# mic-rud/Learned-Compression-of-Point-Cloud-Geometry-and-Attributes

Hardware: AMD Instinct MI355X
Metric: encode+decode Mpoints/sec (higher is better)
Workload: dtype f32

## Files before the change

### include/pcc_hip.h

```cpp
#ifndef PCC_HIP_H
#define PCC_HIP_H

#include <stdint.h>

#ifdef __cplusplus
extern "C" {
#endif

#define PCC_OK 0
#define PCC_ERR_ARG (-1)
#define PCC_ERR_HIP (-2)
#define PCC_ERR_UNSUPPORTED (-3)
#define PCC_ERR_DATA (-4)

#define PCC_ACT_NONE 0
#define PCC_ACT_RELU 1
#define PCC_ACT_LEAKY_RELU 2

int pcc_version(void);
const char* pcc_last_error(void);
int pcc_device_count(void);
int pcc_device_name(int dev, char* out, int out_len);

int64_t pcc_hash_capacity(int64_t n);
// ... 43 lines not shown
int pcc_order_rows_by_mask(const uint32_t* row_mask, const int32_t* coords, int64_t n,
                           int32_t block_log2, int32_t tensor_stride, int32_t* order, uint32_t* group_mask32,
                           void* scratch, int64_t scratch_bytes, void* stream);
int pcc_permute_map_rows(const int32_t* nbr, const int32_t* order, int64_t n, int32_t K, int32_t* nbr_sorted, void* stream);

int64_t pcc_small_map_max(void);
int32_t pcc_small_paths(int32_t mask);
int pcc_small_kernel_map(const int32_t* out_coords, int64_t n_out, const uint64_t* in_keys, const int32_t* in_vals, int64_t in_cap,
                         int32_t ksize, int32_t step, int32_t sign, int32_t* nbr, uint32_t* row_mask, int32_t* order,
                         uint32_t* group_mask32, void* scratch, int64_t scratch_bytes, void* stream);

int64_t pcc_conv_packed_elems(int32_t K, int32_t cin, int32_t cout);
int pcc_conv_pack_weights(const float* w, int32_t K, int32_t cin, int32_t cout, float* w_packed,
                          void* stream);
int pcc_conv_fwd(const float* fin, int64_t n_in, int32_t cin, const float* w, const float* w_packed,
                 const float* bias, const int32_t* nbr, const int32_t* order,
                 const uint32_t* group_mask32, int32_t K, float* fout, int64_t n_out, int32_t cout,
                 int32_t act, const float* film, const float* residual, void* stream);

int64_t pcc_conv_small_max(int64_t workgroups);

int pcc_conv_kernel_name(int32_t mode, int64_t n_in, int32_t cin, int32_t cout, int64_t n_out, int32_t K, int32_t has_nbr,
                         char* buf, int32_t len);

int64_t pcc_conv_packed_elems_bf16(int32_t K, int32_t cin, int32_t cout);
int pcc_conv_pack_weights_bf16(const float* w, int32_t K, int32_t cin, int32_t cout, uint16_t* w_packed, void* stream);
int pcc_conv_fwd_bf16(const uint16_t* fin, int64_t n_in, int32_t cin, const uint16_t* w_packed, const float* bias,
                      const int32_t* nbr, const int32_t* order, const uint32_t* group_mask32, int32_t K, float* fout,
                      int64_t n_out, int32_t cout, int32_t act, const float* film, const float* residual, void* stream);

int pcc_epilogue_fwd(const float* c, const float* film, const float* residual, int64_t n, int32_t channels, int32_t act,
                     float* out, void* stream);
int pcc_epilogue_bwd(const float* dout, const float* c, const float* film, int64_t n, int32_t channels, int32_t act,
                     float* dc, float* dfilm, void* stream);

int64_t pcc_cast_colsum_scratch_elems(int32_t channels);
int pcc_cast_colsum(const float* x, int64_t n, int32_t channels, uint16_t* out_bf16, float* colsum, float* scratch,
                    int64_t scratch_elems, void* stream);

int64_t pcc_conv_packed_elems_x3(int32_t K, int32_t cin, int32_t cout);
int pcc_conv_pack_weights_x3(const float* w, int32_t K, int32_t cin, int32_t cout, uint16_t* w_packed, void* stream);
int pcc_conv_fwd_x3(const float* fin, int64_t n_in, int32_t cin, const uint16_t* w_packed, const float* bias,
                    const int32_t* nbr, const int32_t* order, const uint32_t* group_mask32, int32_t K, float* fout,
                    int64_t n_out, int32_t cout, int32_t act, const float* film, const float* residual, void* stream);

int pcc_im2col_thin(const float* fin, int32_t cin, const int32_t* nbr, int64_t n_out, int32_t K, float* out, int32_t k2,
// ... 146 lines not shown
```

### learned-compression-of-point-cloud-geometry-and-attributes_amd/_build.py

```python
import os
import subprocess

_HERE = os.path.dirname(os.path.abspath(__file__))
SO_PATH = os.path.join(_HERE, "libpcc_hip.so")

NO_SCRATCH = {
    "conv": ("conv_small_kernel", "conv_mfma_buf_kernel", "conv_mfma_kernel"),
    "rans_lanes": ("rans_lanes_encode_kernel", "rans_lanes_pack_kernel", "rans_lanes_decode_kernel"),
    "chconv": ("chconv_kernel",),
    "augment": ("jitter_partial_kernel", "jitter_mean_kernel", "jitter_apply_kernel", "first_rows_clear_kernel",
                "first_rows_insert_kernel", "first_rows_flag_kernel", "first_rows_finalize_kernel"),
    "normals": ("estimate_normals_kernel",),
    "voxelize": ("first_rows_clear_kernel", "first_rows_insert_kernel", "first_rows_flag_kernel", "first_rows_finalize_kernel",
                 "voxelize_accumulate_kernel"),
    "raht": ("raht_plan_kernel", "raht_step_kernel", "raht_fold_kernel"),
}


def build(force=False):
    args = ["make", "-s", "-C", os.path.join(_HERE, "csrc"), "-j4"]
    if force:
        subprocess.check_call(args + ["clean"])
    subprocess.check_call(args)
    for stem, kernels in NO_SCRATCH.items():
        check_kernel_resources(os.path.join(_HERE, "build", stem + ".resources.txt"), kernels)
    check_small_kernel_lds_reads()
    return SO_PATH


def check_small_kernel_lds_reads(obj=None):
# ... 94 lines not shown
```

### learned-compression-of-point-cloud-geometry-and-attributes_amd/csrc/conv.hip

```cpp
#include <stdlib.h>

#include <type_traits>

#include "common.h"

namespace pcc {

typedef float f32x2 __attribute__((ext_vector_type(2)));
typedef float f32x4 __attribute__((ext_vector_type(4)));
typedef __bf16 bf16x8 __attribute__((ext_vector_type(8)));

struct ConvArgs {
    const float* fin;
    const float* w;
    const float* wp;
    const float* bias;
    const int32_t* nbr;
    const int32_t* order;
    const uint32_t* gmask;
    float* fout;
    const float* film;
    const float* residual;
    int64_t n_in, n_out;
    int cin, cout, coutp, K, act;
};

__device__ __forceinline__ float apply_act(float v, int act) {
    if (act == PCC_ACT_RELU) return v > 0.0f ? v : 0.0f;
    if (act == PCC_ACT_LEAKY_RELU) return v > 0.0f ? v : 0.01f * v;
    return v;
}

__device__ __forceinline__ float conv_bias(const ConvArgs& a, int col) { return a.bias ? a.bias[col] : 0.0f; }

__device__ __forceinline__ void conv_store(const ConvArgs& a, int64_t row, int col, float acc, float bcol) {
    float v = acc + bcol;
    if (a.film) {
        const float* fr = a.film + row * (2 * (int64_t)a.cout);
        v = v * fr[col] + fr[a.cout + col];
    }
    v = apply_act(v, a.act);
    if (a.residual) v += a.residual[row * a.cout + col];
    a.fout[row * a.cout + col] = v;
}

__global__ __launch_bounds__(256) void pack_weights_kernel(const float* __restrict__ w, int K, int cin, int cout,
                                                           int cinp, int coutp, float* __restrict__ wp) {
// ... 164 lines not shown
        else if (live == 2u) block(std::integral_constant<unsigned, 2u>{});
    }
}

template <int MT, int NT>
__device__ __forceinline__ void conv_store_tiles(const ConvArgs& a, const f32x16 (&acc)[MT][NT], int64_t pos0, int col0, int h) {
#pragma unroll
    for (int m = 0; m < MT; ++m) {
#pragma unroll
        for (int n = 0; n < NT; ++n) {
            const int col = col0 + 32 * n;
            if (col >= a.cout) continue;
            const float bcol = conv_bias(a, col);
#pragma unroll
            for (int reg = 0; reg < 16; ++reg) {
                const int64_t pos = pos0 + 32 * m + 4 * h + mfma32_row(reg);
                if (pos >= a.n_out) continue;
                conv_store(a, a.order ? a.order[pos] : pos, col, acc[m][n][reg], bcol);
            }
        }
    }
}

template <int BM, int BN, int WAVES_M, int WAVES_N, bool HAS_NBR>
__global__ __launch_bounds__(256) void conv_mfma_kernel(const ConvArgs a) {
    constexpr int RPT = BM / 32;
    constexpr int WM = BM / WAVES_M, WN = BN / WAVES_N;
    constexpr int MT = WM / 32, NT = WN / 32;
    constexpr int A_LD = A_LD_DMA;
    constexpr int A_ELEMS = BM * A_LD;
    constexpr int W_ELEMS = 8 * BN * 4;
    constexpr int W_LOADS = (8 * BN) / 256;
    static_assert(WAVES_M * WAVES_N == 4 && MT >= 1 && NT >= 1 && W_LOADS >= 1, "bad tiling");

    extern __shared__ __attribute__((aligned(16))) float smem[];
    float* As = smem;
    float* Ws = smem + 2 * A_ELEMS;

    const int t = threadIdx.x;
    const int lane = t & 63, wid = t >> 6;
    const int r = lane & 31, h = lane >> 5;
    const int wrow = (wid / WAVES_N) * WM, wcol = (wid % WAVES_N) * WN;

    const int ntiles_n = a.coutp / BN;
    const int64_t tile = blockIdx.x / ntiles_n;
    const int nt = blockIdx.x - (int)(tile * ntiles_n);
// ... 106 lines not shown
            compute(cur, k);
            __syncthreads();
            if (!has_next) break;
            if (advance) { k = nk; rem = rem2; knext = kn2; }
            c = nc;
            cur ^= 1;
        }
    }

    conv_store_tiles(a, acc, row0 + wrow, nt * BN + wcol + r, h);
}

constexpr uint32_t BUF_OOB = 0xFFFFF000u;
[[maybe_unused]] constexpr uint32_t BUF_FLAGS = 0x00020000u;

template <int I, int N, class F>
__device__ __forceinline__ void static_for(F&& f) {
    if constexpr (I < N) {
        f(std::integral_constant<int, I>{});
        static_for<I + 1, N>(f);
    }
}

template <int BM, int BN, int WAVES_M, int WAVES_N, int CCH, bool HAS_NBR, bool BF16 = false, bool X3 = false>
__global__ __launch_bounds__(256) void conv_mfma_buf_kernel(const ConvArgs a) {
#if defined(__HIP_DEVICE_COMPILE__)
    constexpr int RPT = BM / 32;
    constexpr int WM = BM / WAVES_M, WN = BN / WAVES_N;
    constexpr int MT = WM / 32, NT = WN / 32;
    constexpr int A_ELEMS = BM * 32;
    constexpr int W_ELEMS = (X3 ? 12 : 8) * BN * 4;
    constexpr int W_LOADS = ((X3 ? 12 : 8) * BN) / 256;
    static_assert(WAVES_M * WAVES_N == 4 && MT >= 1 && MT <= 2 && NT >= 1 && W_LOADS >= 1, "bad tiling");
    static_assert(!(BF16 && X3), "one operand mode at a time");
    constexpr int ESZ = BF16 ? 2 : 4;

    extern __shared__ __attribute__((aligned(16))) float smem[];
    float* As = smem;
    float* Ws = smem + 2 * A_ELEMS;

    const int t = threadIdx.x;
    const int lane = t & 63, wid = t >> 6;
    const int r = lane & 31, h = lane >> 5;
    const int wrow = (wid / WAVES_N) * WM, wcol = (wid % WAVES_N) * WN;

    const int ntiles_n = a.coutp / BN;
    const int64_t tile = blockIdx.x / ntiles_n;
    const int nt = blockIdx.x - (int)(tile * ntiles_n);
// ... 167 lines not shown
                }
                compute(std::integral_constant<int, buf>{}, live);
                __syncthreads();
            });
            const bool more = knext >= 0;
            k = more ? knext : k;
            rem = rem2;
            return more;
        };

        load_idx(k);
        set_src(true);
        dma(k, std::integral_constant<int, 0>{}, std::integral_constant<int, 0>{});
        load_idx(rem ? __builtin_ctz(rem) : k);
        __syncthreads();
        while (true) {
            if (!offset_body(std::integral_constant<int, 0>{})) break;
            if constexpr (CCH & 1) {
                if (!offset_body(std::integral_constant<int, 1>{})) break;
            }
        }
    }

    conv_store_tiles(a, acc, row0 + wrow, nt * BN + wcol + r, h);
#endif
}

template <int SC, int NS>
constexpr int conv_small_lds_bytes() { return (NS * SC * (32 * 32 + 8 * 32 * 4) + 32 * 32) * (int)sizeof(float); }

template <int SC, int NS>
__global__ __launch_bounds__(512) void conv_small_kernel(const ConvArgs a) {
#if defined(__HIP_DEVICE_COMPILE__)
    constexpr int A_STAGE = SC * 32 * 32;
    constexpr int W_STAGE = SC * 8 * 32 * 4;
    constexpr int STAGE = A_STAGE + W_STAGE;
    constexpr int DMAS = 2 * SC;
    static_assert(NS >= 2 && (NS - 1) * DMAS <= 63, "vmcnt is a 6-bit counter");
    extern __shared__ __attribute__((aligned(16))) float smem[];
    int* idx_s = reinterpret_cast<int*>(smem + NS * STAGE);

    const int t = threadIdx.x;
    const int lane = t & 63;
    const int wave_u = __builtin_amdgcn_readfirstlane(t >> 6);
    const int K = a.K;
    const int ntiles_n = a.coutp / 32;
    const int64_t tile = blockIdx.x / ntiles_n;
// ... 272 lines not shown
        for (int u = 0; u < 9; ++u)
            if (idx[u] >= 0) {
#pragma unroll
                for (int c = 0; c < COUT; ++c) acc[c] += v[u][c];
            }
    }
    float* o = out + (row0 + threadIdx.x) * COUT;
#pragma unroll
    for (int c = 0; c < COUT; ++c) o[c] = apply_act(acc[c] + (bias ? bias[c] : 0.0f), act);
}

enum ConvMode { CONV_F32 = 0, CONV_BF16 = 1, CONV_X3 = 2 };
static const char* const CONV_ENTRY[] = {"pcc_conv_fwd", "pcc_conv_fwd_bf16", "pcc_conv_fwd_x3"};
static const char* const CONV_TAG[] = {"", "[bf16]", "[x3]"};

enum ConvFamily { FAM_THIN, FAM_SMALL, FAM_BUF, FAM_GLOBAL };

struct ConvPlan {
    ConvFamily family;
    int bm, bn, wm, wn;
    int cch;
    int sc, ns;
    int cpt;
};

constexpr int64_t FILL_WGS = 768;
constexpr int64_t ROW32_MAX_WGS = 3000;

static inline int round_up32(int v) { return (v + 31) / 32 * 32; }

static bool fits_buffer_path(const ConvArgs& a) {
    const uint64_t lim = BUF_OOB;
    return (uint64_t)a.n_in * a.cin * 4 <= lim && (uint64_t)a.n_out * a.K * 4 <= lim && (uint64_t)a.K * a.cin * a.coutp * 4 <= lim;
}

static int conv_path() {
    static int path = -1;
    if (path < 0) { const char* e = getenv("PCC_CONV_PATH"); path = (e && e[0] == 'g') ? 1 : 0; }
    return path;
}

static int64_t g_small_max = -1;
static int64_t small_max_value() {
    if (g_small_max < 0) { const char* e = getenv("PCC_CONV_SMALL_MAX"); g_small_max = e ? atoll(e) : 640; }
    return g_small_max;
}

static bool thin_cin(int cin) {
    for (int c : {1, 2, 3, 4, 6, 8, 12, 16, 24})
        if (cin == c) return true;
    return false;
}

static int check_shape(const ConvArgs& a, ConvMode mode, const char* who) {
    PCC_REQUIRE(a.K >= 1 && a.K <= 27, "%s: K=%d out of range", who, a.K);
    if (mode == CONV_F32) PCC_REQUIRE(a.cin % 32 != 0 || a.cin <= 256, "%s: MFMA path supports cin <= 256 (got %d)", who, a.cin);
    if (mode == CONV_BF16) PCC_REQUIRE(a.cin % 64 == 0 && a.cin <= 256, "%s: cin must be a multiple of 64 up to 256 (got %d)", who, a.cin);
    if (mode == CONV_X3) PCC_REQUIRE(a.cin % 32 == 0 && a.cin <= 256, "%s: cin must be a multiple of 32 up to 256 (got %d)", who, a.cin);
    PCC_REQUIRE(a.nbr != nullptr || (a.K == 1 && a.n_in == a.n_out), "%s: nbr == NULL needs K == 1 and n_in == n_out", who);
    return PCC_OK;
}

static int plan_conv(const ConvArgs& a, ConvMode mode, ConvPlan& p, const char* who) {
    p = ConvPlan{};
    if (mode == CONV_F32 && a.cin % 32 != 0) {
        if (!thin_cin(a.cin)) {
            pcc::set_error("%s: unsupported cin=%d (need a multiple of 32 or one of 1,2,3,4,6,8,12,16,24)", who, a.cin);
            return PCC_ERR_UNSUPPORTED;
        }
        const size_t lds = (size_t)a.K * a.cin * a.cout * sizeof(float);
        PCC_REQUIRE(lds <= 160 * 1024, "conv(thin): weights %zu B exceed the 160 KB of LDS (cin=%d cout=%d K=%d)", lds, a.cin, a.cout, a.K);
        p.family = FAM_THIN;
        p.cpt = (a.cout % 8 == 0) ? 8 : (a.cout % 4 == 0) ? 4 : (a.cout % 2 == 0) ? 2 : 1;
        return PCC_OK;
    }
    const bool wide = a.coutp % 128 == 0;
    p.family = FAM_BUF;
    p.cch = a.cin / (mode == CONV_BF16 ? 64 : 32);
    if (mode == CONV_F32) {
        const bool buffer = conv_path() == 0 && fits_buffer_path(a);
        const int64_t wgs32 = ((a.n_out + 31) / 32) * (a.coutp / 32);
        if (a.nbr && buffer && wgs32 <= small_max_value() * (wide ? 1 : 2)) {
            p.family = FAM_SMALL;
            p.sc = (p.cch % 4 == 0 && wgs32 <= 256) ? 4 : p.cch % 2 == 0 ? 2 : 1;
            p.ns = p.sc == 1 ? 8 : 3;
            return PCC_OK;
        }
        if (!buffer) p.family = FAM_GLOBAL;
    } else if (mode == CONV_BF16) {
        PCC_REQUIRE((uint64_t)a.n_in * a.cin * 2 <= BUF_OOB && (uint64_t)a.n_out * a.K * 4 <= BUF_OOB,
                    "%s: operands of 4 GiB and more are not supported", who);
    } else {
        PCC_REQUIRE((uint64_t)a.n_in * a.cin * 4 <= BUF_OOB && (uint64_t)a.n_out * a.K * 4 <= BUF_OOB &&
                    (uint64_t)a.K * a.cin * a.coutp * 6 <= BUF_OOB, "%s: operands of 4 GiB and more are not supported", who);
    }
    const int64_t wgs128 = ((a.n_out + 63) / 64) * (a.coutp / 128);
    auto tile = [&](int bm, int bn, int wm, int wn) { p.bm = bm; p.bn = bn; p.wm = wm; p.wn = wn; return PCC_OK; };
    if (wide && wgs128 < FILL_WGS) return tile(64, 64, 2, 2);
    if (wide && mode == CONV_F32 && wgs128 < ROW32_MAX_WGS) return tile(32, 128, 1, 4);
    if (wide) return tile(64, 128, 2, 2);
    if (a.coutp % 64 == 0) return mode == CONV_X3 ? tile(64, 64, 2, 2) : tile(128, 64, 2, 2);
    if (mode != CONV_X3) return tile(128, 32, 4, 1);
    pcc::set_error("%s: cout=%d not supported (output width rounded up to 32 must be a multiple of 64)", who, a.cout);
    return PCC_ERR_UNSUPPORTED;
}

template <auto KERN>
static int launch(int64_t blocks, int threads, size_t lds, size_t lds_limit, const ConvArgs& a, hipStream_t st) {
    static bool limit_set = false;
    if (lds_limit && !limit_set) {
        PCC_CHECK_HIP(hipFuncSetAttribute(reinterpret_cast<const void*>(KERN), hipFuncAttributeMaxDynamicSharedMemorySize, (int)lds_limit));
        limit_set = true;
    }
    PCC_REQUIRE(blocks < (1ll << 31), "conv: grid too large");
    hipLaunchKernelGGL(KERN, dim3((unsigned)blocks), dim3(threads), lds, st, a);
    PCC_LAUNCH_CHECK();
    return PCC_OK;
}

template <ConvMode M, int BM, int BN, int WM, int WN, int CCH>
static int launch_buf(int64_t blocks, const ConvArgs& a, hipStream_t st) {
    constexpr bool BF16 = M == CONV_BF16, X3 = M == CONV_X3;
    if constexpr (BF16 && CCH > 4) {
        return PCC_ERR_UNSUPPORTED;
    } else {
        constexpr int lds = conv_lds_bytes<BM, BN, X3>();
        return a.nbr ? launch<conv_mfma_buf_kernel<BM, BN, WM, WN, CCH, true, BF16, X3>>(blocks, 256, lds, lds, a, st)
                     : launch<conv_mfma_buf_kernel<BM, BN, WM, WN, CCH, false, BF16, X3>>(blocks, 256, lds, lds, a, st);
    }
}

// ... 11 lines not shown
        case 1: return launch_buf<M, BM, BN, WM, WN, 1>(blocks, a, st);
        case 2: return launch_buf<M, BM, BN, WM, WN, 2>(blocks, a, st);
        case 3: return launch_buf<M, BM, BN, WM, WN, 3>(blocks, a, st);
        case 4: return launch_buf<M, BM, BN, WM, WN, 4>(blocks, a, st);
        case 5: return launch_buf<M, BM, BN, WM, WN, 5>(blocks, a, st);
        case 6: return launch_buf<M, BM, BN, WM, WN, 6>(blocks, a, st);
        case 7: return launch_buf<M, BM, BN, WM, WN, 7>(blocks, a, st);
        case 8: return launch_buf<M, BM, BN, WM, WN, 8>(blocks, a, st);
        default: return PCC_ERR_UNSUPPORTED;
    }
}

template <ConvMode M>
static int launch_tile(const ConvPlan& p, const ConvArgs& a, hipStream_t st) {
    if (p.bm == 64 && p.bn == 64) return launch_mfma<M, 64, 64, 2, 2>(p, a, st);
    if (p.bm == 64 && p.bn == 128) return launch_mfma<M, 64, 128, 2, 2>(p, a, st);
    if constexpr (M == CONV_F32)
        if (p.bm == 32) return launch_mfma<M, 32, 128, 1, 4>(p, a, st);
    if constexpr (M != CONV_X3) {
        if (p.bn == 64) return launch_mfma<M, 128, 64, 2, 2>(p, a, st);
        if (p.bn == 32) return launch_mfma<M, 128, 32, 4, 1>(p, a, st);
    }
    return PCC_ERR_UNSUPPORTED;
}

template <int SC, int NS>
static int launch_small(const ConvArgs& a, hipStream_t st) {
    constexpr int lds = conv_small_lds_bytes<SC, NS>();
    return launch<conv_small_kernel<SC, NS>>(((a.n_out + 31) / 32) * (a.coutp / 32), 512, lds, lds, a, st);
}

template <int CIN>
static int launch_thin(const ConvPlan& p, const ConvArgs& a, hipStream_t st) {
    const size_t lds = (size_t)a.K * CIN * a.cout * sizeof(float);
    const unsigned nb = blocks_for(a.n_out * (a.cout / p.cpt), 256, lds >= 4096 ? 2048u : (1u << 20));
    const size_t limit = lds > 64 * 1024 ? 160 * 1024 : 0;
    if (p.cpt == 8) return launch<conv_thin_kernel<CIN, 8>>(nb, 256, lds, limit, a, st);
    if (p.cpt == 4) return launch<conv_thin_kernel<CIN, 4>>(nb, 256, lds, limit, a, st);
    if (p.cpt == 2) return launch<conv_thin_kernel<CIN, 2>>(nb, 256, lds, limit, a, st);
    return launch<conv_thin_kernel<CIN, 1>>(nb, 256, lds, limit, a, st);
}

static int launch_thin_cin(const ConvPlan& p, const ConvArgs& a, hipStream_t st) {
    switch (a.cin) {
        case 1: return launch_thin<1>(p, a, st);
        case 2: return launch_thin<2>(p, a, st);
// ... 120 lines not shown
    else if (K == 27 && al16 && cout == 3) PCC_GS27(3);
    else if (K == 27 && al16 && cout == 4) PCC_GS27(4);
    else
#undef PCC_GS27
        hipLaunchKernelGGL(gather_sum_kernel, dim3(blocks_for(n_out * cout, 256, 1 << 20)), dim3(256), 0, as_stream(stream),
                           scores, ld, nbr, K, cout, bias, out, n_out, act);
    PCC_LAUNCH_CHECK();
    return PCC_OK;
}

int64_t pcc_conv_small_max(int64_t workgroups) {
    const int64_t before = small_max_value();
    if (workgroups >= 0) g_small_max = workgroups;
    return before;
}

int pcc_conv_fwd(const float* fin, int64_t n_in, int32_t cin, const float* w, const float* w_packed, const float* bias,
                 const int32_t* nbr, const int32_t* order, const uint32_t* group_mask32, int32_t K, float* fout,
                 int64_t n_out, int32_t cout, int32_t act, const float* film, const float* residual, void* stream) {
    return conv_fwd(CONV_F32, {fin, w, w_packed, bias, nbr, order, group_mask32, fout, film, residual, n_in, n_out, cin, cout,
                               round_up32(cout), K, act}, stream);
}

int pcc_conv_kernel_name(int32_t mode, int64_t n_in, int32_t cin, int32_t cout, int64_t n_out, int32_t K, int32_t has_nbr,
                         char* buf, int32_t len) {
    PCC_REQUIRE(mode >= CONV_F32 && mode <= CONV_X3, "pcc_conv_kernel_name: bad mode %d", mode);
    static const int32_t any_map = 0;
    ConvArgs a = {};
    a.nbr = has_nbr ? &any_map : nullptr;
    a.n_in = n_in; a.n_out = n_out; a.cin = cin; a.cout = cout; a.coutp = round_up32(cout); a.K = K;
    const ConvMode m = ConvMode(mode);
    ConvPlan p;
    if (check_shape(a, m, CONV_ENTRY[m]) != PCC_OK || plan_conv(a, m, p, CONV_ENTRY[m]) != PCC_OK) return PCC_ERR_UNSUPPORTED;
    if (buf == nullptr) return PCC_OK;
    const char* tf = has_nbr ? "true" : "false";
    int n;
    if (p.family == FAM_THIN) n = snprintf(buf, len, "conv_thin_kernel<%d, %d>", cin, p.cpt);
    else if (p.family == FAM_SMALL) n = snprintf(buf, len, "conv_small_kernel<%d, %d>", p.sc, p.ns);
    else if (p.family == FAM_GLOBAL) n = snprintf(buf, len, "conv_mfma_kernel<%d, %d, %d, %d, %s>", p.bm, p.bn, p.wm, p.wn, tf);
    else n = snprintf(buf, len, "conv_mfma_buf_kernel%s<%d, %d, %d, %d, %d, %s>", CONV_TAG[m], p.bm, p.bn, p.wm, p.wn, p.cch, tf);
    PCC_REQUIRE(n < len, "pcc_conv_kernel_name: %d bytes do not hold the name", len);
    return PCC_OK;
}

}
```

### learned-compression-of-point-cloud-geometry-and-attributes_amd/sparse.py

```python
import ctypes
import functools
import math
import weakref

import os

import torch
import torch.nn as nn

from . import _lib, _threads
from ._lib import PCC, check, ptr

ACT_NONE, ACT_RELU, ACT_LRELU = PCC.ACT_NONE, PCC.ACT_RELU, PCC.ACT_LEAKY_RELU


def _require_cuda(t):
    if not t.is_cuda:
        raise RuntimeError("libpcc_hip operators need tensors on an MI355X device (got a CPU tensor); "
                           "there is no CPU fallback")


COORD_PROFILER = None


# ... 543 lines not shown
    ev.record()
    return ev


def _prof_end(ev0, name, cin, cout, pairs, n_out, gmask=None):
    if PROFILER is None:
        return
    ev1 = None
    if ev0 is not None:
        ev1 = torch.cuda.Event(enable_timing=True)
        ev1.record()
    PROFILER.append((name, cin, cout, pairs, n_out, ev0, ev1, gmask))


_MFMA_VISIT = (0, 4, 1, 5, 2, 6, 3, 7)


def _thin_im2col_forward(x_feats, in_map, out_map, layer, ksize, transposed, act, film, residual, out_channels):
    L = _lib.lib()
    w2p, bias, k2, cout = layer.im2col_weights(out_channels)
    nbr, _, pairs = in_map.kernel_map(out_map, ksize, transposed)
    n_out, K, cin = out_map.n, ksize ** 3, x_feats.shape[1]
    dev = x_feats.device
    x2 = torch.empty((n_out, k2), dtype=torch.float32, device=dev)
    out = torch.empty((n_out, cout), dtype=torch.float32, device=dev)
    ev0 = _prof_begin()
    ev = _cp_begin()
    check(L.pcc_im2col_thin(ptr(x_feats), cin, ptr(nbr), n_out, K, ptr(x2), k2, _lib.stream()))
    _cp_end(ev, "im2col_thin", n_out, lambda: 4 * K * n_out + 4 * cin * int(pairs) + 4 * k2 * n_out)
    check(L.pcc_conv_fwd(ptr(x2), n_out, k2, None, ptr(w2p), ptr(bias), None, None, None, 1, ptr(out), n_out, cout, act, ptr(film),
                         ptr(residual), _lib.stream()))
    _prof_end(ev0, f"thin_im2col<{cin}>", cin, cout, pairs, n_out)
    return out


def _narrow_head_forward(x_feats, in_map, out_map, layer, ksize, transposed, act, out_channels):
    L = _lib.lib()
    w_r, wp_r, bias, K, cout = layer.narrow_weights(out_channels)
    n_in, cin = x_feats.shape
    n_out = out_map.n
    nbr, _, pairs = in_map.kernel_map(out_map, ksize, transposed)
    ld = K * cout
    scores = torch.empty((n_in, ld), dtype=torch.float32, device=x_feats.device)
    out = torch.empty((n_out, cout), dtype=torch.float32, device=x_feats.device)
    ev0 = _prof_begin()
    check(L.pcc_conv_fwd(ptr(x_feats), n_in, cin, ptr(w_r), ptr(wp_r), None, None, None, None, 1, ptr(scores), n_in, ld,
                         ACT_NONE, None, None, _lib.stream()))
    ev = _cp_begin()
    check(L.pcc_gather_sum_fwd(ptr(scores), ld, ptr(nbr), K, cout, ptr(bias), ptr(out), n_out, act, _lib.stream()))
    _cp_end(ev, "gather_sum", n_out, lambda: 4 * K * n_out + 4 * cout * int(pairs) + 4 * cout * n_out)
    _prof_end(ev0, f"narrow_head<{cin}>", cin, cout, pairs, n_out)
    return out


def set_conv_small_max(workgroups):
    return int(_lib.lib().pcc_conv_small_max(int(workgroups)))


NARROW_HEAD_MAX_COUT = 4

CHECK_EXPECTED_COUNTS = os.environ.get("PCC_CHECK_COUNTS", "0") == "1"
ORDER_BLOCK_LOG2 = int(os.environ.get("PCC_ORDER_BLOCK_LOG2", "-1"))

INFER_BF16 = os.environ.get("PCC_INFER_BF16", "0") == "1"


def set_infer_bf16(enabled):
    global INFER_BF16
    INFER_BF16 = bool(enabled)


INFER_X3 = os.environ.get("PCC_INFER_X3", "0") == "1"


def set_infer_x3(enabled):
    global INFER_X3
    INFER_X3 = bool(enabled)


GATE_LOG = None


PROFILER = None
PROFILER_MIN_ROWS = 65536


MODE_F32, MODE_BF16, MODE_X3 = 0, 1, 2


def conv_kernel_name(mode, n_in, cin, cout, n_out, K, has_nbr):
    buf = ctypes.create_string_buffer(128)
    check(_lib.lib().pcc_conv_kernel_name(mode, n_in, cin, cout, n_out, K, int(has_nbr), buf, len(buf)))
    return buf.value.decode()


def launch_mode(bf16, x3, n_in, cin, cout, n_out, K, has_nbr):
    if bf16 and _plan_takes(MODE_BF16, n_in, cin, cout, n_out, K, has_nbr):
        return MODE_BF16
    if x3 and _plan_takes(MODE_X3, n_in, cin, cout, n_out, K, has_nbr):
        return MODE_X3
    return MODE_F32


@functools.lru_cache(maxsize=4096)
def _plan_takes(mode, n_in, cin, cout, n_out, K, has_nbr):
    return _lib.lib().pcc_conv_kernel_name(mode, n_in, cin, cout, n_out, K, int(has_nbr), None, 0) == 0


def launch_conv(mode, feats, w, wp, bias, nbr, order, gmask, out, act=ACT_NONE, film=None, residual=None):
    L = _lib.lib()
# ... 198 lines not shown

    def plan(self):
        hit = self.__dict__.get("_plan")
        if hit is not None and hit[0] == len(self):
            return hit[1]
        steps = []
        mods = list(self)
        i = 0
        while i < len(mods):
            m = mods[i]
            assert isinstance(m, _ConvBase), f"unexpected module {type(m)} at {i}"
            act = ACT_NONE
            if i + 1 < len(mods) and isinstance(mods[i + 1], MinkowskiReLU):
                act = mods[i + 1].act
                i += 1
            steps.append((m, act))
            i += 1
        self.__dict__["_plan"] = (len(self), steps)
        return steps

    def forward(self, x, last_film=None, last_residual=None, last_out_map=None, last_out_channels=None):
        steps = self.plan()
        last_j = len(steps) - 1
        for j, (m, act) in enumerate(steps):
            if j == last_j:
                x = m.forward(x, act, last_film, last_residual, last_out_map, last_out_channels)
            else:
                x = m.forward(x, act)
        return x


class MinkowskiPruning(nn.Module):

    def forward(self, x, mask):
        coords, feats, _, _ = compact_rows(mask.to(torch.uint8), x.C, x.F)
        return SparseTensor(feats, coordinate_map=CoordMap(coords, x.map.stride, nbatch=x.map._nbatch))
```

Measured before the change: 9.057.

## Fuse narrow head into conv epilogue and gather thin-cin inputs inside conv kernel

Adds a head-fused variant of the buffered MFMA conv kernel. Its epilogue keeps the activated output tile in LDS and multiplies it by the narrow head's weights, so the wide intermediate features never go to global memory and the separate head GEMM launch is dropped. It also adds a thin-cin gather kernel that reads neighbour features directly into LDS, which removes the im2col matrix materialisation and one kernel launch. Both paths are enabled by default through a fusion mask. The cost is extra LDS and register pressure, synchronisations in the epilogue, and more complex planning.

```diff
diff --git a/include/pcc_hip.h b/include/pcc_hip.h
--- a/include/pcc_hip.h
+++ b/include/pcc_hip.h
@@ -89,6 +89,16 @@
 
 int pcc_conv_kernel_name(int32_t mode, int64_t n_in, int32_t cin, int32_t cout, int64_t n_out, int32_t K, int32_t has_nbr,
                          char* buf, int32_t len);
+
+int pcc_conv_head_fwd(const float* fin, int64_t n_in, int32_t cin, const float* w_packed, const float* bias, const int32_t* nbr,
+                      const int32_t* order, const uint32_t* group_mask32, int32_t K, float* fout, int64_t n_out, int32_t cout,
+                      int32_t act, const float* head_w_packed, int32_t head_ld, float* scores, void* stream);
+
+int pcc_conv_thin_fwd(const float* fin, int64_t n_in, int32_t cin, const float* w2_packed, const float* bias, const int32_t* nbr,
+                      int32_t K, float* fout, int64_t n_out, int32_t cout, int32_t act, const float* film, const float* residual,
+                      float* matrix, void* stream);
+
+int32_t pcc_conv_fusion(int32_t mask);
 
 int64_t pcc_conv_packed_elems_bf16(int32_t K, int32_t cin, int32_t cout);
 int pcc_conv_pack_weights_bf16(const float* w, int32_t K, int32_t cin, int32_t cout, uint16_t* w_packed, void* stream);
diff --git a/learned-compression-of-point-cloud-geometry-and-attributes_amd/_build.py b/learned-compression-of-point-cloud-geometry-and-attributes_amd/_build.py
--- a/learned-compression-of-point-cloud-geometry-and-attributes_amd/_build.py
+++ b/learned-compression-of-point-cloud-geometry-and-attributes_amd/_build.py
@@ -5,7 +5,7 @@
 SO_PATH = os.path.join(_HERE, "libpcc_hip.so")
 
 NO_SCRATCH = {
-    "conv": ("conv_small_kernel", "conv_mfma_buf_kernel", "conv_mfma_kernel"),
+    "conv": ("conv_small_kernel", "conv_mfma_buf_kernel", "conv_mfma_kernel", "conv_thin_gather_kernel"),
     "rans_lanes": ("rans_lanes_encode_kernel", "rans_lanes_pack_kernel", "rans_lanes_decode_kernel"),
     "chconv": ("chconv_kernel",),
     "augment": ("jitter_partial_kernel", "jitter_mean_kernel", "jitter_apply_kernel", "first_rows_clear_kernel",
diff --git a/learned-compression-of-point-cloud-geometry-and-attributes_amd/csrc/conv.hip b/learned-compression-of-point-cloud-geometry-and-attributes_amd/csrc/conv.hip
--- a/learned-compression-of-point-cloud-geometry-and-attributes_amd/csrc/conv.hip
+++ b/learned-compression-of-point-cloud-geometry-and-attributes_amd/csrc/conv.hip
@@ -23,6 +23,12 @@
     const float* residual;
     int64_t n_in, n_out;
     int cin, cout, coutp, K, act;
+};
+
+struct ConvHeadArgs : ConvArgs {
+    const float* hwp;
+    float* scores;
+    int hld, hldp;
 };
 
 __device__ __forceinline__ float apply_act(float v, int act) {
@@ -233,6 +239,68 @@
     }
 }
 
+template <int BM, int BN, int MT, int NT>
+__device__ __forceinline__ void conv_head_epilogue(const ConvHeadArgs& a, const f32x16 (&acc)[MT][NT], int64_t row0, int wrow,
+                                                   int wcol) {
+    extern __shared__ __attribute__((aligned(16))) float smem[];
+    constexpr int CH = BN / 32;
+    constexpr int RT = BM / 32;
+    static_assert(RT <= 4 && (BM * BN + CH * 1024) * (int)sizeof(float) <= conv_lds_bytes<BM, BN>(), "head epilogue: LDS");
+    float* Wh = smem + BM * BN;
+    const int t = threadIdx.x;
+    const int lane = t & 63, r = lane & 31, h = lane >> 5;
+    const int wid = __builtin_amdgcn_readfirstlane(t >> 6);
+    __syncthreads();
+#pragma unroll
+    for (int m = 0; m < MT; ++m) {
+#pragma unroll
+        for (int n = 0; n < NT; ++n) {
+            const int col = wcol + 32 * n + r;
+            const float bcol = conv_bias(a, col);
+            float* img = smem + (col >> 5) * (BM * 32) + (col & 3);
+            const int slot = (col & 31) >> 2;
+#pragma unroll
+            for (int reg = 0; reg < 16; ++reg) {
+                const int row = wrow + 32 * m + 4 * h + mfma32_row(reg);
+                const float v = apply_act(acc[m][n][reg] + bcol, a.act);
+                img[row * 32 + ((slot ^ ((row >> 1) & 7)) << 2)] = v;
+                const int64_t pos = row0 + row;
+                if (a.fout && pos < a.n_out) a.fout[(a.order ? a.order[pos] : pos) * a.cout + col] = v;
+            }
+        }
+    }
+    uint32_t a_addr[CH][4];
+#pragma unroll
+    for (int c = 0; c < CH; ++c)
+#pragma unroll
+        for (int kk = 0; kk < 4; ++kk) a_addr[c][kk] = (uint32_t)(c * BM * 32 * 4) + a_frag_offset(32 * wid + r, h, kk);
+    const uint32_t w_addr = (uint32_t)((BM * BN + (h * 32 + r) * 4) * 4);
+    const int ntile = a.hldp >> 5;
+    for (int n2 = 0; n2 < ntile; ++n2) {
+#pragma unroll
+        for (int c = 0; c < CH; ++c) {
+            const int g = c * 8 + (t >> 5);
+            *reinterpret_cast<f32x4*>(Wh + (g * 32 + (t & 31)) * 4) =
+                *reinterpret_cast<const f32x4*>(a.hwp + ((int64_t)g * a.hldp + n2 * 32 + (t & 31)) * 4);
+        }
+        __syncthreads();
+        if (wid < RT) {
+            f32x16 sc[1][1] = {};
+#pragma unroll
+            for (int c = 0; c < CH; ++c) mfma_step<1u, 32, false>(sc, a_addr[c], w_addr + (uint32_t)(c * 1024 * 4));
+            const int col = n2 * 32 + r;
+            if (col < a.hld) {
+#pragma unroll
+                for (int reg = 0; reg < 16; ++reg) {
+                    const int64_t pos = row0 + 32 * wid + 4 * h + mfma32_row(reg);
+                    if (pos < a.n_out) a.scores[(a.order ? a.order[pos] : pos) * a.hld + col] = sc[0][0][reg] + 0.0f;
+                }
+            }
+        }
+        if (n2 + 1 < ntile) __syncthreads();
+    }
+}
+
 template <int BM, int BN, int WAVES_M, int WAVES_N, bool HAS_NBR>
 __global__ __launch_bounds__(256) void conv_mfma_kernel(const ConvArgs a) {
     constexpr int RPT = BM / 32;
@@ -385,8 +453,116 @@
     }
 }
 
-template <int BM, int BN, int WAVES_M, int WAVES_N, int CCH, bool HAS_NBR, bool BF16 = false, bool X3 = false>
-__global__ __launch_bounds__(256) void conv_mfma_buf_kernel(const ConvArgs a) {
+template <int BM, int BN, int WAVES_M, int WAVES_N, int CCH, int CIN, int MT, int NT>
+__device__ __forceinline__ void thin_gather_loop(const ConvArgs& a, int64_t row0, int nt, int wrow, int wcol, f32x16 (&acc)[MT][NT]) {
+#if defined(__HIP_DEVICE_COMPILE__)
+    constexpr int RPT = BM / 32;
+    constexpr int A_ELEMS = BM * 32;
+    constexpr int W_ELEMS = 8 * BN * 4;
+    constexpr int W_LOADS = (8 * BN) / 256;
+    constexpr int NK = CIN >= 8 ? 1 : CIN == 4 ? 2 : 4;
+    constexpr int KT = 27;
+    static_assert(CIN == 1 || CIN == 2 || CIN == 4 || CIN == 8, "thin gather: cin");
+    extern __shared__ __attribute__((aligned(16))) float smem[];
+    float* As = smem;
+    float* Ws = smem + 2 * A_ELEMS;
+    const int t = threadIdx.x;
+    const int lane = t & 63, wid = t >> 6;
+    const int r = lane & 31, h = lane >> 5;
+    const int wave_u = __builtin_amdgcn_readfirstlane(wid);
+
+    __amdgpu_buffer_rsrc_t rsrc_w = __builtin_amdgcn_make_buffer_rsrc(const_cast<float*>(a.wp), 0, (int)((uint32_t)(CCH * 32) * a.coutp * 4),
+                                                                      BUF_FLAGS);
+    uint32_t w_voff[W_LOADS];
+#pragma unroll
+    for (int j = 0; j < W_LOADS; ++j) {
+        const int f = t + 256 * j;
+        const int g = f / BN, col = f - g * BN;
+        w_voff[j] = (uint32_t)((g * a.coutp + nt * BN + col) * 16);
+    }
+    const uint32_t w_cstride = 8u * a.coutp * 16;
+    auto dma_w = [&](int c, int buf) {
+#pragma unroll
+        for (int j = 0; j < W_LOADS; ++j)
+            __builtin_amdgcn_raw_ptr_buffer_load_lds(rsrc_w, (lds_ptr_t)(Ws + buf * W_ELEMS + (wave_u * 64 + 256 * j) * 4), 16, w_voff[j],
+                                                     (uint32_t)c * w_cstride, 0, 0);
+    };
+
+    int idx[RPT][CCH][NK], lbase[RPT];
+#pragma unroll
+    for (int i = 0; i < RPT; ++i) {
+        const int grow = wid * (BM / 4) + 8 * i + (lane >> 3);
+        const int q = (t & 7) ^ ((grow >> 1) & 7);
+        lbase[i] = 8 * (q >> 1) + (q & 1);
+        const int64_t pos = row0 + grow;
+#pragma unroll
+        for (int c = 0; c < CCH; ++c)
+#pragma unroll
+            for (int j = 0; j < NK; ++j) {
+                const int k = (32 * c + lbase[i] + 2 * j * (4 / NK)) / CIN;
+                idx[i][c][j] = (pos < a.n_out && k < KT) ? a.nbr[pos * KT + k] : -1;
+            }
+    }
+    auto gather = [&](int c, f32x4 (&v)[RPT]) {
+#pragma unroll
+        for (int i = 0; i < RPT; ++i)
+#pragma unroll
+            for (int s = 0; s < 4; ++s) {
+                const int id = idx[i][c][s / (4 / NK)];
+                const int ci = (32 * c + lbase[i] + 2 * s) % CIN;
+                const float x = a.fin[(int64_t)(id >= 0 ? id : 0) * CIN + ci];
+                v[i][s] = id >= 0 ? x : 0.0f;
+            }
+    };
+    auto put = [&](int buf, const f32x4 (&v)[RPT]) {
+#pragma unroll
+        for (int i = 0; i < RPT; ++i) *reinterpret_cast<f32x4*>(As + buf * A_ELEMS + (wid * RPT + i) * 256 + lane * 4) = v[i];
+    };
+
+    uint32_t a_addr[2][4], w_addr[2];
+#pragma unroll
+    for (int b = 0; b < 2; ++b) {
+#pragma unroll
+        for (int kk = 0; kk < 4; ++kk) a_addr[b][kk] = (uint32_t)(b * A_ELEMS * 4) + a_frag_offset(wrow + r, h, kk);
+        w_addr[b] = (uint32_t)((2 * A_ELEMS + b * W_ELEMS + (h * BN + wcol + r) * 4) * 4);
+    }
+
+    f32x4 v[RPT];
+    dma_w(0, 0);
+    gather(0, v);
+    put(0, v);
+    __syncthreads();
+    static_for<0, CCH>([&](auto cc) {
+        constexpr int c = decltype(cc)::value;
+        constexpr int buf = c & 1;
+        if constexpr (c + 1 < CCH) {
+            dma_w(c + 1, buf ^ 1);
+            gather(c + 1, v);
+        }
+        mfma_step<(1u << MT) - 1u, BN, false>(acc, a_addr[buf], w_addr[buf]);
+        if constexpr (c + 1 < CCH) put(buf ^ 1, v);
+        __syncthreads();
+    });
+#endif
+}
+
+template <int BM, int BN, int WAVES_M, int WAVES_N, int CCH, int CIN>
+__global__ __launch_bounds__(256) void conv_thin_gather_kernel(const ConvArgs a) {
+    constexpr int WM = BM / WAVES_M, WN = BN / WAVES_N;
+    constexpr int MT = WM / 32, NT = WN / 32;
+    static_assert(WAVES_M * WAVES_N == 4 && MT >= 1 && MT <= 2 && NT >= 1, "bad tiling");
+    const int lane = threadIdx.x & 63, wid = threadIdx.x >> 6;
+    const int wrow = (wid / WAVES_N) * WM, wcol = (wid % WAVES_N) * WN;
+    const int ntiles_n = a.coutp / BN;
+    const int64_t tile = blockIdx.x / ntiles_n;
+    const int nt = blockIdx.x - (int)(tile * ntiles_n);
+    f32x16 acc[MT][NT] = {};
+    thin_gather_loop<BM, BN, WAVES_M, WAVES_N, CCH, CIN>(a, tile * BM, nt, wrow, wcol, acc);
+    conv_store_tiles(a, acc, tile * BM + wrow, nt * BN + wcol + (lane & 31), lane >> 5);
+}
+
+template <int BM, int BN, int WAVES_M, int WAVES_N, int CCH, bool HAS_NBR, bool BF16 = false, bool X3 = false, bool HEAD = false>
+__global__ __launch_bounds__(256) void conv_mfma_buf_kernel(const std::conditional_t<HEAD, ConvHeadArgs, ConvArgs> a) {
 #if defined(__HIP_DEVICE_COMPILE__)
     constexpr int RPT = BM / 32;
     constexpr int WM = BM / WAVES_M, WN = BN / WAVES_N;
@@ -600,7 +776,8 @@
         }
     }
 
-    conv_store_tiles(a, acc, row0 + wrow, nt * BN + wcol + r, h);
+    if constexpr (HEAD) conv_head_epilogue<BM, BN>(a, acc, row0, wrow, wcol);
+    else conv_store_tiles(a, acc, row0 + wrow, nt * BN + wcol + r, h);
 #endif
 }
 
@@ -919,6 +1096,7 @@
     int cch;
     int sc, ns;
     int cpt;
+    bool fused;
 };
 
 constexpr int64_t FILL_WGS = 768;
@@ -935,6 +1113,12 @@
     static int path = -1;
     if (path < 0) { const char* e = getenv("PCC_CONV_PATH"); path = (e && e[0] == 'g') ? 1 : 0; }
     return path;
+}
+
+static int g_fusion = -1;
+static int fusion_value() {
+    if (g_fusion < 0) { const char* e = getenv("PCC_CONV_FUSION"); g_fusion = e ? (atoi(e) & 3) : 3; }
+    return g_fusion;
 }
 
 static int64_t g_small_max = -1;
@@ -958,7 +1142,7 @@
     return PCC_OK;
 }
 
-static int plan_conv(const ConvArgs& a, ConvMode mode, ConvPlan& p, const char* who) {
+static int plan_conv(const ConvArgs& a, ConvMode mode, ConvPlan& p, const char* who, bool want_head = false) {
     p = ConvPlan{};
     if (mode == CONV_F32 && a.cin % 32 != 0) {
         if (!thin_cin(a.cin)) {
@@ -992,7 +1176,12 @@
                     (uint64_t)a.K * a.cin * a.coutp * 6 <= BUF_OOB, "%s: operands of 4 GiB and more are not supported", who);
     }
     const int64_t wgs128 = ((a.n_out + 63) / 64) * (a.coutp / 128);
-    auto tile = [&](int bm, int bn, int wm, int wn) { p.bm = bm; p.bn = bn; p.wm = wm; p.wn = wn; return PCC_OK; };
+    auto tile = [&](int bm, int bn, int wm, int wn) {
+        p.bm = bm; p.bn = bn; p.wm = wm; p.wn = wn;
+        p.fused = want_head && mode == CONV_F32 && p.family == FAM_BUF && bn == a.coutp && a.cout == a.coutp && a.nbr &&
+                 (p.cch == 1 || p.cch == 2 || p.cch == 4) && !a.film && !a.residual && (fusion_value() & 1);
+        return PCC_OK;
+    };
     if (wide && wgs128 < FILL_WGS) return tile(64, 64, 2, 2);
     if (wide && mode == CONV_F32 && wgs128 < ROW32_MAX_WGS) return tile(32, 128, 1, 4);
     if (wide) return tile(64, 128, 2, 2);
@@ -1002,8 +1191,8 @@
     return PCC_ERR_UNSUPPORTED;
 }
 
-template <auto KERN>
-static int launch(int64_t blocks, int threads, size_t lds, size_t lds_limit, const ConvArgs& a, hipStream_t st) {
+template <auto KERN, class Args>
+static int launch(int64_t blocks, int threads, size_t lds, size_t lds_limit, const Args& a, hipStream_t st) {
     static bool limit_set = false;
     if (lds_limit && !limit_set) {
         PCC_CHECK_HIP(hipFuncSetAttribute(reinterpret_cast<const void*>(KERN), hipFuncAttributeMaxDynamicSharedMemorySize, (int)lds_limit));
@@ -1061,6 +1250,57 @@
         if (p.bn == 32) return launch_mfma<M, 128, 32, 4, 1>(p, a, st);
     }
     return PCC_ERR_UNSUPPORTED;
+}
+
+template <int BM, int BN, int WM, int WN>
+static int launch_head_tile(const ConvPlan& p, const ConvHeadArgs& a, hipStream_t st) {
+    const int64_t blocks = (a.n_out + BM - 1) / BM;
+    constexpr int lds = conv_lds_bytes<BM, BN>();
+    switch (p.cch) {
+        case 1: return launch<conv_mfma_buf_kernel<BM, BN, WM, WN, 1, true, false, false, true>>(blocks, 256, lds, lds, a, st);
+        case 2: return launch<conv_mfma_buf_kernel<BM, BN, WM, WN, 2, true, false, false, true>>(blocks, 256, lds, lds, a, st);
+        case 4: return launch<conv_mfma_buf_kernel<BM, BN, WM, WN, 4, true, false, false, true>>(blocks, 256, lds, lds, a, st);
+        default: return PCC_ERR_UNSUPPORTED;
+    }
+}
+
+static int launch_head(const ConvPlan& p, const ConvHeadArgs& a, hipStream_t st) {
+    if (p.bm == 64 && p.bn == 128) return launch_head_tile<64, 128, 2, 2>(p, a, st);
+    if (p.bm == 32 && p.bn == 128) return launch_head_tile<32, 128, 1, 4>(p, a, st);
+    if (p.bm == 128 && p.bn == 64) return launch_head_tile<128, 64, 2, 2>(p, a, st);
+    if (p.bm == 128 && p.bn == 32) return launch_head_tile<128, 32, 4, 1>(p, a, st);
+    return PCC_ERR_UNSUPPORTED;
+}
+
+template <int BM, int BN, int WM, int WN>
+static int launch_gather_tile(const ConvArgs& a, hipStream_t st) {
+    const int64_t blocks = (a.n_out + BM - 1) / BM * (a.coutp / BN);
+    constexpr int lds = conv_lds_bytes<BM, BN>();
+    switch (a.cin) {
+        case 1: return launch<conv_thin_gather_kernel<BM, BN, WM, WN, 1, 1>>(blocks, 256, lds, lds, a, st);
+        case 2: return launch<conv_thin_gather_kernel<BM, BN, WM, WN, 2, 2>>(blocks, 256, lds, lds, a, st);
+        case 4: return launch<conv_thin_gather_kernel<BM, BN, WM, WN, 4, 4>>(blocks, 256, lds, lds, a, st);
+        case 8: return launch<conv_thin_gather_kernel<BM, BN, WM, WN, 7, 8>>(blocks, 256, lds, lds, a, st);
+        default: return PCC_ERR_UNSUPPORTED;
+    }
+}
+
+static int launch_gather(const ConvPlan& p, const ConvArgs& a, hipStream_t st) {
+    if (p.bm == 64 && p.bn == 64) return launch_gather_tile<64, 64, 2, 2>(a, st);
+    if (p.bm == 64 && p.bn == 128) return launch_gather_tile<64, 128, 2, 2>(a, st);
+    if (p.bm == 32 && p.bn == 128) return launch_gather_tile<32, 128, 1, 4>(a, st);
+    if (p.bm == 128 && p.bn == 64) return launch_gather_tile<128, 64, 2, 2>(a, st);
+    if (p.bm == 128 && p.bn == 32) return launch_gather_tile<128, 32, 4, 1>(a, st);
+    return PCC_ERR_UNSUPPORTED;
+}
+
+static int plan_thin_gather(int cin, int cout, int64_t n_out, int K, ConvPlan& p, const char* who) {
+    ConvArgs m = {};
+    m.n_in = m.n_out = n_out; m.cin = round_up32(K * cin); m.cout = cout; m.coutp = round_up32(cout); m.K = 1;
+    const int rc = plan_conv(m, CONV_F32, p, who);
+    if (rc != PCC_OK) return rc;
+    p.fused = K == 27 && (cin == 1 || cin == 2 || cin == 4 || cin == 8) && p.family == FAM_BUF && (fusion_value() & 2);
+    return PCC_OK;
 }
 
 template <int SC, int NS>
@@ -1227,8 +1467,87 @@
                                round_up32(cout), K, act}, stream);
 }
 
+int32_t pcc_conv_fusion(int32_t mask) {
+    const int before = fusion_value();
+    if (mask >= 0) g_fusion = mask & 3;
+    return before;
+}
+
+int pcc_conv_head_fwd(const float* fin, int64_t n_in, int32_t cin, const float* w_packed, const float* bias, const int32_t* nbr,
+                      const int32_t* order, const uint32_t* group_mask32, int32_t K, float* fout, int64_t n_out, int32_t cout,
+                      int32_t act, const float* head_w_packed, int32_t head_ld, float* scores, void* stream) {
+    const char* who = "pcc_conv_head_fwd";
+    ConvHeadArgs a = {};
+    a.fin = fin; a.wp = w_packed; a.bias = bias; a.nbr = nbr; a.order = order; a.gmask = group_mask32; a.fout = fout;
+    a.n_in = n_in; a.n_out = n_out; a.cin = cin; a.cout = cout; a.coutp = round_up32(cout); a.K = K; a.act = act;
+    a.hwp = head_w_packed; a.scores = scores; a.hld = head_ld; a.hldp = round_up32(head_ld);
+    int rc = check_shape(a, CONV_F32, who);
+    if (rc != PCC_OK) return rc;
+    PCC_REQUIRE(act >= 0 && act <= 2, "%s: bad activation %d", who, act);
+    PCC_REQUIRE(cin % 32 == 0 && cout % 32 == 0 && cout <= 256, "%s: cin=%d and cout=%d must be multiples of 32 (cout <= 256)", who, cin, cout);
+    PCC_REQUIRE(head_ld >= 1 && head_w_packed != nullptr && scores != nullptr, "%s: head weights and scores required", who);
+    PCC_REQUIRE(w_packed != nullptr && ((reinterpret_cast<uintptr_t>(fin) | reinterpret_cast<uintptr_t>(w_packed) |
+                                         reinterpret_cast<uintptr_t>(head_w_packed)) & 15) == 0,
+                "%s: fin, w_packed and head_w_packed must be 16-byte aligned", who);
+    if (n_out <= 0) return PCC_OK;
+    ConvPlan p;
+    if ((rc = plan_conv(a, CONV_F32, p, who, true)) != PCC_OK) return rc;
+    if (p.fused) return launch_head(p, a, as_stream(stream));
+    PCC_REQUIRE(fout != nullptr, "%s: this shape runs as two launches and needs fout", who);
+    if ((rc = conv_fwd(CONV_F32, a, stream)) != PCC_OK) return rc;
+    return conv_fwd(CONV_F32, {fout, nullptr, head_w_packed, nullptr, nullptr, nullptr, nullptr, scores, nullptr, nullptr, n_out, n_out,
+                               cout, head_ld, round_up32(head_ld), 1, PCC_ACT_NONE}, stream);
+}
+
+int pcc_conv_thin_fwd(const float* fin, int64_t n_in, int32_t cin, const float* w2_packed, const float* bias, const int32_t* nbr,
+                      int32_t K, float* fout, int64_t n_out, int32_t cout, int32_t act, const float* film, const float* residual,
+                      float* matrix, void* stream) {
+    const char* who = "pcc_conv_thin_fwd";
+    PCC_REQUIRE(K >= 1 && K <= 27 && cin >= 1 && cin <= 16 && K * cin <= 256, "%s: bad shape (K=%d cin=%d)", who, K, cin);
+    PCC_REQUIRE(cout >= 32 && cout % 32 == 0, "%s: cout=%d must be a multiple of 32", who, cout);
+    PCC_REQUIRE(act >= 0 && act <= 2, "%s: bad activation %d", who, act);
+    PCC_REQUIRE(nbr != nullptr && w2_packed != nullptr && (reinterpret_cast<uintptr_t>(w2_packed) & 15) == 0,
+                "%s: nbr and 16-byte aligned packed weights required", who);
+    if (n_out <= 0) return PCC_OK;
+    const int k2 = round_up32(K * cin);
+    ConvPlan p;
+    int rc = plan_thin_gather(cin, cout, n_out, K, p, who);
+    if (rc != PCC_OK) return rc;
+    if (p.fused)
+        return launch_gather(p, {fin, nullptr, w2_packed, bias, nbr, nullptr, nullptr, fout, film, residual, n_in, n_out, cin, cout,
+                                 round_up32(cout), K, act}, as_stream(stream));
+    PCC_REQUIRE(matrix != nullptr, "%s: this shape runs as two launches and needs the [n_out, %d] matrix buffer", who, k2);
+    if ((rc = pcc_im2col_thin(fin, cin, nbr, n_out, K, matrix, k2, stream)) != PCC_OK) return rc;
+    return conv_fwd(CONV_F32, {matrix, nullptr, w2_packed, bias, nullptr, nullptr, nullptr, fout, film, residual, n_out, n_out, k2, cout,
+                               round_up32(cout), 1, act}, stream);
+}
+
 int pcc_conv_kernel_name(int32_t mode, int64_t n_in, int32_t cin, int32_t cout, int64_t n_out, int32_t K, int32_t has_nbr,
                          char* buf, int32_t len) {
+    if (mode == 4) {
+        ConvPlan p;
+        if (!has_nbr || K < 1 || K > 27 || cin < 1 || cin > 16 || cout % 32 != 0 ||
+            plan_thin_gather(cin, cout, n_out, K, p, "pcc_conv_thin_fwd") != PCC_OK || !p.fused)
+            return PCC_ERR_UNSUPPORTED;
+        if (buf == nullptr) return PCC_OK;
+        const int n = snprintf(buf, len, "conv_thin_gather_kernel<%d, %d, %d, %d, %d, %d>", p.bm, p.bn, p.wm, p.wn, p.cch, cin);
+        PCC_REQUIRE(n < len, "pcc_conv_kernel_name: %d bytes do not hold the name", len);
+        return PCC_OK;
+    }
+    if (mode == 3) {
+        static const int32_t a_map = 0;
+        ConvArgs a = {};
+        a.nbr = has_nbr ? &a_map : nullptr;
+        a.n_in = n_in; a.n_out = n_out; a.cin = cin; a.cout = cout; a.coutp = round_up32(cout); a.K = K;
+        ConvPlan p;
+        if (cin % 32 != 0 || check_shape(a, CONV_F32, "pcc_conv_head_fwd") != PCC_OK ||
+            plan_conv(a, CONV_F32, p, "pcc_conv_head_fwd", true) != PCC_OK || !p.fused)
+            return PCC_ERR_UNSUPPORTED;
+        if (buf == nullptr) return PCC_OK;
+        const int n = snprintf(buf, len, "conv_mfma_buf_kernel[head]<%d, %d, %d, %d, %d, true>", p.bm, p.bn, p.wm, p.wn, p.cch);
+        PCC_REQUIRE(n < len, "pcc_conv_kernel_name: %d bytes do not hold the name", len);
+        return PCC_OK;
+    }
     PCC_REQUIRE(mode >= CONV_F32 && mode <= CONV_X3, "pcc_conv_kernel_name: bad mode %d", mode);
     static const int32_t any_map = 0;
     ConvArgs a = {};
diff --git a/learned-compression-of-point-cloud-geometry-and-attributes_amd/sparse.py b/learned-compression-of-point-cloud-geometry-and-attributes_amd/sparse.py
--- a/learned-compression-of-point-cloud-geometry-and-attributes_amd/sparse.py
+++ b/learned-compression-of-point-cloud-geometry-and-attributes_amd/sparse.py
@@ -589,8 +589,14 @@
     nbr, _, pairs = in_map.kernel_map(out_map, ksize, transposed)
     n_out, K, cin = out_map.n, ksize ** 3, x_feats.shape[1]
     dev = x_feats.device
+    out = torch.empty((n_out, cout), dtype=torch.float32, device=dev)
+    if _plan_takes(MODE_THIN, x_feats.shape[0], cin, cout, n_out, K, True):
+        ev0 = _prof_begin()
+        check(L.pcc_conv_thin_fwd(ptr(x_feats), x_feats.shape[0], cin, ptr(w2p), ptr(bias), ptr(nbr), K, ptr(out), n_out, cout, act,
+                                  ptr(film), ptr(residual), None, _lib.stream()))
+        _prof_end(ev0, f"thin_gather<{cin}>", cin, cout, pairs, n_out)
+        return out
     x2 = torch.empty((n_out, k2), dtype=torch.float32, device=dev)
-    out = torch.empty((n_out, cout), dtype=torch.float32, device=dev)
     ev0 = _prof_begin()
     ev = _cp_begin()
     check(L.pcc_im2col_thin(ptr(x_feats), cin, ptr(nbr), n_out, K, ptr(x2), k2, _lib.stream()))
@@ -620,7 +626,50 @@
     return out
 
 
+def head_fusable(layer, x_feats, n_out, head, head_out_channels=None):
+    if head.stride != 1 or head.transposed or head.kernel_size <= 1 or layer.kernel_size <= 1 or INFER_BF16 or INFER_X3:
+        return False
+    cin, cout = layer.in_channels, layer.out_channels
+    hc = head.out_channels if head_out_channels is None else head_out_channels
+    if cin % 32 or cout % 32 or head.in_channels != cout or hc > NARROW_HEAD_MAX_COUT or x_feats.shape[1] != cin:
+        return False
+    if torch.is_grad_enabled() and (layer.kernel.requires_grad or head.kernel.requires_grad or x_feats.requires_grad):
+        return False
+    return _plan_takes(MODE_HEAD, x_feats.shape[0], cin, cout, n_out, layer.kernel_size ** 3, True)
+
+
+def conv_head_forward(x_feats, in_map, out_map, layer, act, head, head_act, head_out_channels=None):
+    L = _lib.lib()
+    w, wp, bias = layer.weights()
+    w_r, wp_r, hbias, hK, hcout = head.narrow_weights(head_out_channels)
+    n_in, cin = x_feats.shape
+    cout, n_out, K = w.shape[-1], out_map.n, layer.kernel_size ** 3
+    nbr, order, gmask, pairs = in_map.conv_map(out_map, layer.kernel_size, layer.transposed, cin)
+    hnbr, _, hpairs = out_map.kernel_map(out_map, head.kernel_size, False)
+    ld = hK * hcout
+    scores = torch.empty((n_out, ld), dtype=torch.float32, device=x_feats.device)
+    out = torch.empty((n_out, hcout), dtype=torch.float32, device=x_feats.device)
+    timed = PROFILER is not None and n_out >= PROFILER_MIN_ROWS
+    ev0 = _prof_begin(timed)
+    check(L.pcc_conv_head_fwd(ptr(x_feats), n_in, cin, ptr(wp), ptr(bias), ptr(nbr), ptr(order), ptr(gmask), K, None, n_out, cout,
+                              act, ptr(wp_r), ld, ptr(scores), _lib.stream()))
+    _prof_end(ev0, ("conv", MODE_HEAD, n_in, K, True), cin, cout, pairs, n_out, gmask)
+    ev0 = _prof_begin()
+    ev = _cp_begin()
+    check(L.pcc_gather_sum_fwd(ptr(scores), ld, ptr(hnbr), hK, hcout, ptr(hbias), ptr(out), n_out, head_act, _lib.stream()))
+    _cp_end(ev, "gather_sum", n_out, lambda: 4 * hK * n_out + 4 * hcout * int(hpairs) + 4 * hcout * n_out)
+    _prof_end(ev0, f"narrow_head<{cout}>", cout, hcout, hpairs, n_out)
+    return out
+
+
+def set_conv_fusion(mask):
+    _plan_takes.cache_clear()
+    return int(_lib.lib().pcc_conv_fusion(int(mask)))
+
+
 def set_conv_small_max(workgroups):
+    if workgroups >= 0:
+        _plan_takes.cache_clear()
     return int(_lib.lib().pcc_conv_small_max(int(workgroups)))
 
 
@@ -653,6 +702,8 @@
 
 
 MODE_F32, MODE_BF16, MODE_X3 = 0, 1, 2
+MODE_HEAD = 3
+MODE_THIN = 4
 
 
 def conv_kernel_name(mode, n_in, cin, cout, n_out, K, has_nbr):
@@ -897,7 +948,24 @@
     def forward(self, x, last_film=None, last_residual=None, last_out_map=None, last_out_channels=None):
         steps = self.plan()
         last_j = len(steps) - 1
+        skip = False
         for j, (m, act) in enumerate(steps):
+            if skip:
+                skip = False
+                continue
+            if j < last_j and m.kernel_size > 1 and m.out_channels % 32 == 0:
+                head, head_act = steps[j + 1]
+                hoc = last_out_channels if j + 1 == last_j else None
+                if ((head.out_channels if hoc is None else hoc) <= NARROW_HEAD_MAX_COUT
+                        and (j + 1 < last_j or (last_film is None and last_residual is None and last_out_map is None))):
+                    out_map = m.output_map(x.map)
+                    if head_fusable(m, x.F, out_map.n, head, hoc):
+                        feats = conv_head_forward(x.F, x.map, out_map, m, act, head, head_act, hoc)
+                        x = SparseTensor._wrap(feats, out_map)
+                        skip = True
+                    else:
+                        x = m.forward(x, act, None, None, out_map)
+                    continue
             if j == last_j:
                 x = m.forward(x, act, last_film, last_residual, last_out_map, last_out_channels)
             else:
```

After: 9.147, median of 6. About the same (+1.0%).
